# abiswas-odu/Disco

Hardware: AMD Instinct MI355X
Metric: overlaps/sec (BuildGraph stage), 150 bp reads (higher is better)
Workload: dtype u64; 1 GPU; 50000000 x 150 bp synthetic reads, 30x of 50 x 5000000 bp uniform-random contigs, both strands, error-free, min-overlap 40 (k=39), transitive reduction on, seed 42; reads=50000000, read_len=150, min_overlap=40, parallelism=1 GPU, e_pre=903537181, e_out=45314794, n_contained=4685156, cap_bind_sites=0, asymmetric_pairs=0, probes=5550000000, kmer_hits=2220071992

## Files before the change

### disco_amd/csrc/disco_hip.hip

```cpp
#include <hip/hip_runtime.h>
#include <rocprofiler-sdk-roctx/roctx.h>

#include <algorithm>
#include <atomic>
#include <chrono>
#include <cstdarg>
#include <cstdio>
#include <cstdlib>
#include <cstring>
#include <functional>
#include <fcntl.h>
#include <sys/mman.h>
#include <sys/stat.h>
#include <unistd.h>
#include <string>
#include <memory>
#include <thread>
#include <map>
#include <mutex>
#include <queue>
#include <vector>

#include "../../include/disco_hip.h"
#include "../../include/disco_hip_test.h"
// ... 412 lines not shown
            return DISCO_OK;
        }
    }
    tl_pass.dev_allocs++;
    HIPCHK(c, hipMalloc((void **)p, bytes));
    c->hbm_bytes += bytes;
    c->hbm_peak = std::max(c->hbm_peak, c->hbm_bytes);
    return DISCO_OK;
}

template <typename T>
static void dev_free(disco_ctx *c, T **p, size_t count)
{
    if (*p) {
        if (c->arena.owns(*p)) c->arena.release(*p);
        else {
            tl_pass.dev_frees++;
            (void)hipFree(*p);
        }
        c->hbm_bytes -= std::max<size_t>(count, 1) * sizeof(T);
        *p = nullptr;
    }
}

template <typename T>
static void release(disco_ctx *c, DevBuf<T> &b)
{
    dev_free(c, &b.p, b.cap);
    b.cap = 0;
}

template <typename T>
static int ensure(disco_ctx *c, DevBuf<T> &b, u64 need)
{
    if (b.p && need <= b.cap) return DISCO_OK;
    release(c, b);
    CHK(dev_alloc(c, &b.p, need));
    b.cap = std::max<u64>(need, 1);
    return DISCO_OK;
}

template <typename... T>
static int ensure_group(disco_ctx *c, u64 need, u64 size, DevBuf<T> &...b)
{
    if (((need <= b.cap) && ...)) return DISCO_OK;
    (release(c, b), ...);
    int rc = DISCO_OK;
    ((rc = rc == DISCO_OK ? ensure(c, b, size) : rc), ...);
    if (rc != DISCO_OK) (release(c, b), ...);
    return rc;
}

template <typename T>
static int move_keep(disco_ctx *c, DevBuf<T> &b, u64 ncap, u64 used)
{
    DevBuf<T> q;
    CHK(ensure(c, q, ncap));
    if (b.p && used) HIPCHK(c, hipMemcpyAsync(q.p, b.p, used * sizeof(T), hipMemcpyDeviceToDevice, c->stream));
    HIPCHK(c, hipStreamSynchronize(c->stream));
    release(c, b);
    b = q;
    return DISCO_OK;
}

template <typename T>
static int ensure_keep(disco_ctx *c, DevBuf<T> &b, u64 need, u64 used)
{
    if (b.p && need <= b.cap) return DISCO_OK;
    return move_keep(c, b, need + need / 8, used);
}

template <typename T>
static void adopt(disco_ctx *c, DevBuf<T> &b, DevBuf<T> from)
{
    b = from;
    c->hbm_bytes += b.cap * sizeof(T);
}

template <typename T>
static T *disown(disco_ctx *c, DevBuf<T> &b)
{
    T *p = b.p;
    c->hbm_bytes -= b.cap * sizeof(T);
    b = DevBuf<T>();
    return p;
}

static DiscoView view(const disco_ctx *c)
{
    DiscoView v;
    v.reads = c->d_reads;
    v.len = c->d_len;
    v.n = c->n;
    v.S = c->S;
    v.k = c->k;
    v.ks = c->ks;
    v.m = disco_minimizer_len(c->ks);
    if (const char *e = getenv("DISCO_MINIMIZER_LEN")) {
        const int m = atoi(e);
        if (m >= 1 && (m & 1) && m <= v.m && c->ks - m <= 63) v.m = m;
    }
    v.bkt = c->d_bkt;
    v.ent = c->d_ent;
    v.bshift = c->bshift;
    v.q_lo = c->q_lo;
    v.q_hi = c->q_hi;
    v.ctr = c->d_ctr;
    v.wq = c->d_wq;
    v.full = c->two_class ? c->d_full : nullptr;
    v.ovf = c->two_class ? c->d_ovf : nullptr;
    v.long_ids = c->two_class ? c->d_long_ids : nullptr;
    v.n_long = c->two_class ? (u32)c->n_long : 0u;
    v.SL = c->two_class ? c->S_ext : 0;
    v.tailb = c->two_class ? c->tailb : 0;
    return v;
}

static OwnSet own_set(const disco_ctx *c)
{
    OwnSet o;
    o.otab = c->loci ? c->d_otab : nullptr;
    o.me = c->comm ? (u32)c->comm->rank : 0u;
    o.lo = c->q_lo;
    o.hi = c->q_hi;
    o.list = c->loci ? c->d_order_own : nullptr;
    o.n_own = c->loci ? c->n_own : 0;
    o.ids = c->loci ? c->d_own_ids : nullptr;
    return o;
}

static int settle_keys(disco_ctx *c)
{
    if (c->keys_pending) {
        c->keys_pending = false;
        HIPCHK(c, hipStreamWaitEvent(c->stream, c->ev_keys, 0));
    }
    return DISCO_OK;
}

static int env_int(const char *name, int dflt)
{
    const char *e = getenv(name);
    return e ? atoi(e) : dflt;
}

static int wave_grid(const disco_ctx *c, u64 items, int per_cu = 24)
{
    u64 g = (u64)c->n_cu * per_cu;
    if (items < g) g = items;
    return (int)std::max<u64>(g, 1);
}

template <typename K>
static int wq_grid(disco_ctx *c, K kernel, u64 items, const char *env, int cap = 32)
{
    (void)hipMemsetAsync(c->d_wq, 0, sizeof(u64) * WQ_WORDS, c->stream);
    int per_cu = 0;
    if (hipOccupancyMaxActiveBlocksPerMultiprocessor(&per_cu, kernel, 64, 0) != hipSuccess || per_cu <= 0) per_cu = 16;
    if (per_cu > cap) per_cu = cap;
    per_cu = env_int(env, per_cu);
    u64 g = (u64)c->n_cu * per_cu;
    const u64 chunks = (items + WQ_CHUNK - 1) / WQ_CHUNK;
    if (chunks < g) g = chunks;
    return (int)std::max<u64>(g, 1);
}

template <typename K, typename... A>
static void wq_launch(disco_ctx *c, K kernel, u64 items, const char *env, int cap, A... args)
{
    const int g = wq_grid(c, kernel, items, env, cap);
    hipLaunchKernelGGL(kernel, dim3(g), dim3(64), 0, c->stream, args...);
}

static int flat_grid(const disco_ctx *c, u64 items, int block = 256)
{
    u64 g = (items + block - 1) / block;
    u64 cap = (u64)c->n_cu * 16;
    return (int)std::max<u64>(std::min(g, cap), 1);
}

static int read_counters(disco_ctx *c)
{
    HIPCHK(c, hipMemcpyAsync(c->h_ctr, c->d_ctr, sizeof(c->h_ctr), hipMemcpyDeviceToHost, c->stream));
    HIPCHK(c, hipStreamSynchronize(c->stream));
    return DISCO_OK;
}

static int zero_counter(disco_ctx *c, int idx)
{
    HIPCHK(c, hipMemsetAsync(c->d_ctr + idx, 0, sizeof(u64), c->stream));
    return DISCO_OK;
}

template <typename InT, typename OutT>
static int scan_exclusive_on(disco_ctx *c, hipStream_t st, DevBuf<u64> &tile, u64 *total, const InT *in, u64 n, OutT *out, bool write_total, u64 *total_host)
{
    u64 nt = (n + SCAN_TILE - 1) / SCAN_TILE;
    if (nt == 0) nt = 1;
    CHK(ensure(c, tile, nt));
    hipLaunchKernelGGL((scan_tile_sums_kernel<InT>), dim3((unsigned)nt), dim3(SCAN_BLOCK), 0, st, in, n, tile.p);
    hipLaunchKernelGGL(scan_sums_kernel, dim3(1), dim3(1024), 0, st, tile.p, nt, total);
    hipLaunchKernelGGL((scan_apply_kernel<InT, OutT>), dim3((unsigned)nt), dim3(SCAN_BLOCK), 0, st, in, n, tile.p, out);
    if (write_total) hipLaunchKernelGGL((scan_write_total_kernel<OutT>), dim3(1), dim3(1), 0, st, total, out + n);
    HIPCHK(c, hipGetLastError());
    if (total_host) {
        HIPCHK(c, hipMemcpyAsync(total_host, total, sizeof(u64), hipMemcpyDeviceToHost, st));
        HIPCHK(c, hipStreamSynchronize(st));
    }
    return DISCO_OK;
}

template <typename InT, typename OutT>
static int scan_exclusive(disco_ctx *c, const InT *in, u64 n, OutT *out, bool write_total, u64 *total_host)
{
    return scan_exclusive_on<InT, OutT>(c, c->stream, c->d_tile, c->d_total, in, n, out, write_total, total_host);
}

static void drop_edge_records(disco_ctx *c)
{
    c->rec_e_ready = false;
    release(c, c->d_rec_efile);
    release(c, c->d_rec_subs);
    release(c, c->d_rec_efindex);
}
static void drop_contained_records(disco_ctx *c)
{
    c->rec_c_ready = false;
    c->rec_c_n = 0;
    release(c, c->d_rec_cword);
    release(c, c->d_rec_csup);
    release(c, c->d_rec_cfindex);
}

static void free_graph_state(disco_ctx *c)
{
    drop_edge_records(c);
    drop_contained_records(c);
    release(c, c->d_rec_piece[0]);
    release(c, c->d_rec_piece[1]);
    if (c->keys_pending) {
        c->keys_pending = false;
        if (c->ev_keys) (void)hipEventSynchronize(c->ev_keys);
    }
    release(c, c->d_bkt);
    release(c, c->d_ent);
    release(c, c->d_rec);
    release(c, c->d_rec2);
    release(c, c->d_binx);
    release(c, c->d_best);
    release(c, c->d_hits);
    release(c, c->d_row_start);
    release(c, c->d_row_cnt);
    release(c, c->d_big_list);
    release(c, c->d_big_cnt);
    release(c, c->d_slow_list);
    release(c, c->d_runs);
    c->runs_n = 0;
    c->runs_lpr = 0;
    release(c, c->d_contained);
    release(c, c->d_cbits);
    release(c, c->d_dropbits);
    release(c, c->d_drop_node);
    release(c, c->d_drop_key);
    release(c, c->d_adj_ref);
    release(c, c->d_adj_own);
    release(c, c->d_adj_spare);
    release(c, c->d_start_tmp);
    release(c, c->d_ocnt);
    release(c, c->d_okey);
    release(c, c->d_meta_ord);
    release(c, c->d_asked);
    release(c, c->d_oslot);
    release(c, c->d_order_own);
    c->d_order_used = nullptr;
    c->d_adj = nullptr;
    release(c, c->d_extra_cnt);
    release(c, c->d_extra_node);
    release(c, c->d_extra_key);
    release(c, c->d_half);
    release(c, c->d_hcnt);
    release(c, c->d_wide);
    release(c, c->d_n_wide);
    c->adj_total = 0;
    release(c, c->d_out_valid);
    release(c, c->d_ch_comp);
    release(c, c->d_ch_links);
    release(c, c->d_ch_dead);
    release(c, c->d_ch_first);
    release(c, c->d_ch_res_pos);
    release(c, c->d_ch_res_slot);
    c->ch_res_n = 0;
    release(c, c->d_ptext);
    c->ptext_bytes = 0;
    c->ptext_off.clear();
    release(c, c->d_text);
    c->text_bytes = 0;
    release(c, c->d_ctext);
    c->ctext_bytes = 0;
    c->ctext_off.clear();
    c->ch_ready = false;
    release(c, c->d_out_pos);
    release(c, c->d_out_src);
    release(c, c->d_out_ent);
    c->n_out = c->out_used = 0;
    c->flags_pending = false;
    c->adj_imported = false;
    c->T = 0;
    release(c, c->d_x16a);
    release(c, c->d_x16b);
    release(c, c->d_req_flat);
    release(c, c->d_req_s);
    release(c, c->d_req_r);
    release(c, c->d_rdeg_s);
    release(c, c->d_rdeg_r);
    release(c, c->d_rdata_s);
// ... 2527 lines not shown
    if (!c) return DISCO_E_ARG;
    if (c->phase < 5) return fail(c, DISCO_E_STATE, "disco_symmetrize: select edges first");
    HIPCHK(c, hipSetDevice(c->device));
    CHK(twin_check(c, full ? 0 : c->q_lo, full ? c->n : c->q_hi));
    if (n_asym) *n_asym = c->asym_local;
    c->phase = 6;
    return DISCO_OK;
}

int disco_merge_extras(disco_ctx *c)
{
    if (!c) return DISCO_E_ARG;
    if (c->phase < 6) return fail(c, DISCO_E_STATE, "disco_merge_extras: symmetrize first");
    HIPCHK(c, hipSetDevice(c->device));
    return merge_extras(c);
}

int disco_build_edges(disco_ctx *c, uint64_t *n_pre)
{
    if (!c) return DISCO_E_ARG;
    CHK(disco_select_edges(c));
    CHK(disco_symmetrize(c, 1, nullptr));
    CHK(merge_extras(c));
    if (n_pre) *n_pre = c->adj_total / 2;
    return DISCO_OK;
}

int disco_adjacency_size(disco_ctx *c, uint64_t *n_entries)
{
    if (!c || !n_entries) return DISCO_E_ARG;
    if (c->phase < 5) return fail(c, DISCO_E_STATE, "disco_adjacency_size: select edges first");
    *n_entries = c->adj_total;
    return DISCO_OK;
}

int disco_export_adjacency(disco_ctx *c, void *d_deg_u32, void *d_entries_u64)
{
    if (!c || !d_deg_u32) return DISCO_E_ARG;
    if (c->phase < 5 || c->adj_imported) return fail(c, DISCO_E_STATE, "disco_export_adjacency: needs the locally selected edges");
    HIPCHK(c, hipSetDevice(c->device));
    const u64 nq = c->q_hi - c->q_lo;
    ph_begin(c, DISCO_PH_CSR);
    if (nq) hipLaunchKernelGGL(deg_from_ref_kernel, dim3(flat_grid(c, nq)), dim3(256), 0, c->stream, c->d_adj_ref, c->q_lo, c->q_hi, (u32 *)d_deg_u32);
    HIPCHK(c, hipGetLastError());
    if (nq && c->adj_total && d_entries_u64) {
        CHK(ensure(c, c->d_start_tmp, c->n + 1));
        u64 *start = c->d_start_tmp;
        u64 total = 0;
        int rc = scan_exclusive<u32, u64>(c, (const u32 *)d_deg_u32, nq, start, true, &total);
        if (rc == DISCO_OK && total != c->adj_total) rc = fail(c, DISCO_E_STATE, "disco_export_adjacency: degree sum %llu != %llu", (unsigned long long)total, (unsigned long long)c->adj_total);
        if (rc == DISCO_OK) hipLaunchKernelGGL(rows_gather_kernel, dim3(wave_grid(c, nq, 16)), dim3(64), 0, c->stream, c->d_adj, c->d_adj_ref, c->q_lo, c->q_hi, start, (u64 *)d_entries_u64,
                                              (c->phase == 5 && c->prm.max_substitutions != 0) ? 0ull : (u64)ADJ_FLAG);
        hipError_t e = hipStreamSynchronize(c->stream);
        CHK(rc);
        if (e != hipSuccess) return fail(c, DISCO_E_HIP, "disco_export_adjacency: %s", hipGetErrorString(e));
    }
    ph_end(c, DISCO_PH_CSR);
    HIPCHK(c, hipStreamSynchronize(c->stream));
    ph_collect(c);
    return DISCO_OK;
}





int disco_import_adjacency(disco_ctx *c, const void *d_deg_u32_all, const void *d_entries_u64_all, uint64_t n_entries_all)
{
    if (!c || !d_deg_u32_all) return DISCO_E_ARG;
    if (c->phase < 5) return fail(c, DISCO_E_STATE, "disco_import_adjacency: select edges first");
    HIPCHK(c, hipSetDevice(c->device));
    CHK(ensure(c, c->d_start_tmp, c->n + 1));
    u64 *start = c->d_start_tmp;
    u64 total = 0;
    CHK((scan_exclusive<u32, u64>(c, (const u32 *)d_deg_u32_all, c->n, start, true, &total)));
    if (total != n_entries_all)
        return fail(c, DISCO_E_ARG, "disco_import_adjacency: degrees sum to %llu but %llu entries were passed", (unsigned long long)total, (unsigned long long)n_entries_all);
    CHK(ensure(c, c->d_adj_own, total));
    c->d_adj = c->d_adj_own;
    c->adj_total = total;
    if (total) HIPCHK(c, hipMemcpyAsync(c->d_adj, d_entries_u64_all, total * 8, hipMemcpyDeviceToDevice, c->stream));
    if (c->n) hipLaunchKernelGGL(ref_from_start_kernel, dim3(flat_grid(c, c->n)), dim3(256), 0, c->stream, start, (const u32 *)d_deg_u32_all, c->n, c->d_adj_ref);
    HIPCHK(c, hipGetLastError());
    HIPCHK(c, hipStreamSynchronize(c->stream));
    c->adj_imported = true;
    c->tr_big_counted = false;
    c->adj_span = total;
    c->half_complete = false;
    c->phase = 5;
    return DISCO_OK;
}




int disco_transitive_mark(disco_ctx *c)
{
    DISCO_TRACE("disco_transitive_mark");
    if (!c) return DISCO_E_ARG;
    if (c->phase < 6) return fail(c, DISCO_E_STATE, "disco_transitive_mark: build edges first");
    HIPCHK(c, hipSetDevice(c->device));
    const u64 nq = c->q_hi - c->q_lo;
    HIPCHK(c, hipMemsetAsync(c->d_n_big, 0, sizeof(u32), c->stream));
    CHK(zero_counter(c, CTR_OVERFLOW));
    const bool counted_nodes = c->tr_big_counted && c->q_lo == 0 && c->q_hi == c->n && !getenv("DISCO_COUNT_BIG_ROWS");
    const bool tr_small = env_int("DISCO_TR_SMALL", counted_nodes && c->h_ctr[CTR_TR_MID] * 100 <= nq ? 1 : 0) != 0 && counted_nodes;
    if (counted_nodes) {
        const u64 need = c->h_ctr[tr_small ? CTR_TR_MID : CTR_TR_BIG] + 1024;
        if (need > 0xFFFFFFFFull) return fail(c, DISCO_E_CAPACITY, "more than 2^32 big nodes");
        CHK(grow_big_lists(c, need));
    } else
        CHK(ensure_big_cap(c, nullptr, c->d_adj_ref, TR_CAP));
    c->use_half = !getenv("DISCO_NO_HALF");
    const u32 all_flags = (c->adj_imported || !c->use_half || c->q_lo != 0 || c->q_hi != c->n) ? 1u : 0u;
    const bool lists = c->use_half && !all_flags;
    TrArgs a;
    CHK(tr_args_begin(c, &a, lists));
    a.order = (c->d_order_used && c->order_q_lo == c->q_lo && c->order_q_hi == c->q_hi && !c->adj_imported && !getenv("DISCO_TR_NO_ORDER")) ? c->d_order_used : nullptr;
    a.all_flags = all_flags;
    ph_begin(c, DISCO_PH_TRMARK);
    if (nq) wq_launch(c, tr_pick(false, false, tr_small, lists), nq, "DISCO_TR_WAVES", 32, a);
    ph_end(c, DISCO_PH_TRMARK);
    HIPCHK(c, hipGetLastError());
    u32 n_big = 0;
    HIPCHK(c, hipMemcpyAsync(&n_big, c->d_n_big, sizeof(u32), hipMemcpyDeviceToHost, c->stream));
    c->n_wide = 0;
    if (c->use_half) HIPCHK(c, hipMemcpyAsync(&c->n_wide, c->d_n_wide, sizeof(u32), hipMemcpyDeviceToHost, c->stream));
    CHK(read_counters(c));
    ph_collect(c);
    if (c->h_ctr[CTR_OVERFLOW]) return fail(c, DISCO_E_CAPACITY, "transitive marking: big-node list overflow (%u nodes)", n_big);
    if (n_big) {
        CHK(tr_big_nodes(c, &a, n_big, false, "big nodes"));
        if (c->h_ctr[CTR_OVERFLOW]) return fail(c, DISCO_E_CAPACITY, "transitive marking (big nodes): list overflow");
    }
    if (n_big && c->use_half) HIPCHK(c, hipMemcpy(&c->n_wide, c->d_n_wide, sizeof(u32), hipMemcpyDeviceToHost));
    c->flags_pending = false;
    c->phase = 7;
    return DISCO_OK;
}


int disco_emit_edges(disco_ctx *c, uint64_t *n_out)
{
    DISCO_TRACE("disco_emit_edges");
    if (!c) return DISCO_E_ARG;
    if (c->phase < 7) return fail(c, DISCO_E_STATE, "disco_emit_edges: run disco_transitive_mark first");
    HIPCHK(c, hipSetDevice(c->device));
    drop_edge_records(c);
    const u64 nq = c->q_hi - c->q_lo;
    ph_begin(c, DISCO_PH_EMIT);
    const int grid = wq_grid(c, emit_kernel<false>, nq, "DISCO_EMIT_WAVES");
    const u64 n_push = c->dist_active ? c->n_push_r : 0;
    const int grid_push = (int)std::max<u64>(std::min<u64>((n_push + 63) / 64, (u64)c->n_cu * 16), 1);
    const u64 nwaves = (u64)grid * 2 + (n_push ? (u64)grid_push : 0);
    u64 want = std::max<u64>(2 * nq, 1024) + n_push + nwaves * EMIT_CHUNK;
    for (int attempt = 0; attempt < 6; attempt++) {
        CHK(ensure_group(c, want, want, c->d_out_src, c->d_out_ent));
        HIPCHK(c, hipMemsetAsync(c->d_bump, 0, sizeof(u64), c->stream));
        const bool half_emit = c->use_half && c->half_complete;
        const bool dense = half_emit && c->half_selfdel && !c->dist_active;
        if (half_emit && c->half_selfdel && !dense) return fail(c, DISCO_E_STATE, "disco_emit_edges: self-delimiting lists under a communicator");
        c->out_dense = dense;
        if (half_emit && nq) {
            EmitHalfArgs h;
            h.v = view(c);
            h.ref = c->d_adj_ref;
            h.adj = c->d_adj;
            h.half = c->d_half;
            h.hcnt = dense ? nullptr : (const u32 *)c->d_hcnt;
            h.out_src = c->d_out_src;
            h.out_ent = c->d_out_ent;
            h.out_cap = c->d_out_src.cap;
            h.bump = c->d_bump;
            h.local_only = c->dist_active ? 1u : 0u;
            h.own = own_set(c);
            h.order = nullptr;
            if (dense) {
                const int gh = wq_grid(c, emit_half_lists_kernel, (nq + 63) / 64, "DISCO_EMIT_WAVES");
                hipLaunchKernelGGL(emit_half_lists_kernel, dim3(gh), dim3(64), 0, c->stream, h);
            } else {
                const int gh = wq_grid(c, emit_half_kernel, (nq + 63) / 64, "DISCO_EMIT_WAVES");
                hipLaunchKernelGGL(emit_half_kernel, dim3(gh), dim3(64), 0, c->stream, h);
            }
        }
        EmitArgs a;
        a.v = view(c);
        a.ref = c->d_adj_ref;
        a.adj = c->d_adj;
        a.hcnt = half_emit && !dense ? (const u32 *)c->d_hcnt : nullptr;
        a.half = half_emit ? c->d_half : nullptr;
        const bool listed = half_emit && c->n_wide <= c->d_wide.cap;
        a.list = listed ? c->d_wide : nullptr;
        a.n_list = listed ? c->n_wide : 0;
        a.out_src = c->d_out_src;
        a.out_ent = c->d_out_ent;
        a.out_cap = c->d_out_src.cap;
        a.bump = c->d_bump;
        a.local_only = c->dist_active ? 1u : 0u;
        a.own = own_set(c);
        HIPCHK(c, hipMemsetAsync(c->d_wq, 0, sizeof(u64) * WQ_WORDS, c->stream));
        if (nq && !(listed && c->n_wide == 0)) {
            if (dense) hipLaunchKernelGGL(emit_kernel<true>, dim3(grid), dim3(64), 0, c->stream, a);
            else hipLaunchKernelGGL(emit_kernel<false>, dim3(grid), dim3(64), 0, c->stream, a);
        }
        if (n_push) {
            EmitRecvArgs pr;
            pr.items = c->d_push_r;
            pr.n_items = n_push;
            pr.ref = c->d_adj_ref;
            pr.adj = c->d_adj;
            pr.half = c->d_half;
            pr.hcnt = c->d_hcnt;
            pr.out_src = c->d_out_src;
            pr.out_ent = c->d_out_ent;
            pr.out_cap = c->d_out_src.cap;
            pr.bump = c->d_bump;
            pr.wq = c->d_wq;
            HIPCHK(c, hipMemsetAsync(c->d_wq, 0, sizeof(u64) * WQ_WORDS, c->stream));
            hipLaunchKernelGGL(emit_push_recv_kernel, dim3(grid_push), dim3(64), 0, c->stream, pr);
        }
        HIPCHK(c, hipGetLastError());
        u64 used = 0;
        HIPCHK(c, hipMemcpyAsync(&used, c->d_bump, sizeof(u64), hipMemcpyDeviceToHost, c->stream));
        HIPCHK(c, hipStreamSynchronize(c->stream));
        if (used <= c->d_out_src.cap) {
            c->out_used = used;
            break;
        }
        want = used + used / 8 + nwaves * EMIT_CHUNK;
        if (attempt == 5) return fail(c, DISCO_E_CAPACITY, "disco_emit_edges: output buffer could not be sized");
    }
    u64 total = 0;
    if (c->out_dense) {
        total = c->out_used;
        release(c, c->d_out_valid);
        release(c, c->d_out_pos);
    } else if (c->out_used) {
        if (c->out_used > c->d_out_valid.cap || c->out_used + 1 > c->d_out_pos.cap) {
            release(c, c->d_out_valid);
            release(c, c->d_out_pos);
            int rc = ensure(c, c->d_out_valid, c->d_out_src.cap);
            if (rc == DISCO_OK) rc = ensure(c, c->d_out_pos, c->d_out_src.cap + 1);
            if (rc != DISCO_OK) {
                release(c, c->d_out_valid);
                return rc;
            }
        }
        hipLaunchKernelGGL(emit_valid_kernel, dim3(flat_grid(c, c->out_used)), dim3(256), 0, c->stream, c->d_out_src, c->out_used, c->d_out_valid);
        CHK((scan_exclusive<u8, u64>(c, c->d_out_valid, c->out_used, c->d_out_pos, true, nullptr)));
        HIPCHK(c, hipMemcpyAsync(&total, c->d_total, sizeof(u64), hipMemcpyDeviceToHost, c->stream));
    }
    ph_end(c, DISCO_PH_EMIT);
    HIPCHK(c, hipStreamSynchronize(c->stream));
    ph_collect(c);
    c->n_out = total;
    if (n_out) *n_out = total;
    c->phase = 8;
    return DISCO_OK;
}

int disco_transitive_reduce(disco_ctx *c, uint64_t *n_out)
{
    CHK(disco_transitive_mark(c));
    return disco_emit_edges(c, n_out);
}

int disco_run_graph(disco_ctx *c)
{
    DISCO_TRACE("disco_run_graph");
    const bool verbose = getenv("DISCO_VERBOSE") != nullptr;
    auto now = [] { return std::chrono::steady_clock::now(); };
    auto ms = [](std::chrono::steady_clock::time_point a, std::chrono::steady_clock::time_point b) { return std::chrono::duration<double, std::milli>(b - a).count(); };
    auto t0 = now();
    CHK(disco_build_index(c));
    auto t1 = now();
    CHK(disco_probe(c));
    auto t2 = now();
    {
        CHK(ensure(c, c->d_contained, c->n_alloc));
        CHK(ensure(c, c->d_cbits, c->n_alloc / 64 + 1));
        CHK(zero_counter(c, CTR_N_CONTAINED));
        ph_begin(c, DISCO_PH_CONTAIN);
        if (c->n) hipLaunchKernelGGL(contain_flags_kernel, dim3(flat_grid(c, c->n)), dim3(256), 0, c->stream, c->d_best, c->n, c->d_contained, c->d_cbits, c->d_ctr);
        HIPCHK(c, hipGetLastError());
        ph_end(c, DISCO_PH_CONTAIN);
        c->contained_count_pending = true;
        c->phase = 4;
        c->crows_pending = c->cgrp_pending = false;
    }
    auto t3 = now();
    CHK(disco_build_edges(c, nullptr));
    auto t4 = now();
    int rc = disco_transitive_reduce(c, nullptr);
    auto t5 = now();
    if (verbose)
        fprintf(stderr, "[disco] host wall ms: index %.1f probe %.1f contain %.1f edges %.1f reduce %.1f\n", ms(t0, t1), ms(t1, t2), ms(t2, t3), ms(t3, t4), ms(t4, t5));
    return rc;
}

static int ensure_host_len(disco_ctx *c)
{
    std::lock_guard<std::mutex> lk(c->h_len_mu);
    if (c->h_len_ok && c->h_len.size() == c->n) return DISCO_OK;
    c->h_len.resize(c->n);
    if (c->n) HIPCHK(c, hipMemcpy(c->h_len.data(), c->d_len, c->n * 2, hipMemcpyDeviceToHost));
    c->h_len_ok = true;
    return DISCO_OK;
}

int64_t disco_fetch_contained(disco_ctx *c, disco_contained_row *out, uint64_t cap)
{
    DISCO_TRACE("disco_fetch_contained");
    if (!c) return DISCO_E_ARG;
    if (c->phase < 4) return fail(c, DISCO_E_STATE, "disco_fetch_contained: run disco_mark_contained first");
    HIPCHK(c, hipSetDevice(c->device));
    const u64 nc = c->n_contained;
    if (!out) return (int64_t)nc;
    if (cap < nc) return fail(c, DISCO_E_ARG, "disco_fetch_contained: need room for %llu rows", (unsigned long long)nc);
    if (nc == 0) return 0;
    auto decode = [&](auto id_of, const u64 *keys_h, const u32 *lens_h) {
        const u16 *hlen = lens_h ? nullptr : c->h_len.data();
        const u32 kk = (u32)c->k;
        parallel_for(nc, [&, hlen, kk, lens_h](u64 b, u64 e_) {
            for (u64 i = b; i < e_; i++) {
                const u64 key = keys_h[i];
                disco_contained_row &r = out[i];
                r.contained = id_of(i);
                r.super = CKEY_SUPER(key);
                r.j = CKEY_J(key);
                r.type = disco_hit_type(CKEY_SUFFIX(key), CKEY_REV(key));
                r.len2 = lens_h ? (lens_h[i] & 0xFFFFu) : hlen[r.contained];
                r.len1 = lens_h ? (lens_h[i] >> 16) : hlen[r.super];
                u32 orient, off;
                disco_map_type(r.type, r.len1, kk, r.j, &orient, &off);
                r.orient = orient;
                r.start = off;
            }
        });
    };
    CHK(start_contained_rows(c, false));
    if (c->crows_pending && c->crows_n == nc) {
        HIPCHK(c, hipEventSynchronize(c->ev_crows));
        const u64 *hkey = (const u64 *)c->h_crows;
        const u32 *hid = (const u32 *)(hkey + c->crows_hcap);
        decode([hid](u64 i) { return (u64)hid[i]; }, hkey, hid + c->crows_hcap);
        return (int64_t)nc;
    }
    CHK(ensure_host_len(c));
    CHK(settle_keys(c));
    DevBuf<u64> pos, ids, keys;
    std::vector<u64> hid(nc), hkey(nc);
    auto gather = [&]() -> int {
        CHK(ensure(c, pos, c->n + 1));
        CHK(ensure(c, ids, nc));
        CHK(ensure(c, keys, nc));
        CHK((scan_exclusive<u8, u64>(c, c->d_contained, c->n, pos, false, nullptr)));
        hipLaunchKernelGGL(contain_rows_kernel, dim3(flat_grid(c, c->n)), dim3(256), 0, c->stream, c->d_best, c->d_contained, pos, c->n, ids, keys);
        HIPCHK(c, hipMemcpyAsync(hid.data(), ids, nc * 8, hipMemcpyDeviceToHost, c->stream));
        HIPCHK(c, hipMemcpyAsync(hkey.data(), keys, nc * 8, hipMemcpyDeviceToHost, c->stream));
        HIPCHK(c, hipStreamSynchronize(c->stream));
        return DISCO_OK;
    };
    const int grc = gather();
    release(c, pos);
    release(c, ids);
    release(c, keys);
    CHK(grc);
    for (u64 i = 0; i < nc; i++)
        if (CKEY_SUPER(hkey[i]) >= c->n || hid[i] >= c->n)
            return fail(c, DISCO_E_STATE, "disco_fetch_contained: row %llu of %llu: read %llu has the key %llx (no containing read)", (unsigned long long)i, (unsigned long long)nc,
                        (unsigned long long)hid[i], (unsigned long long)hkey[i]);
    decode([&hid](u64 i) { return hid[i]; }, hkey.data(), nullptr);
    return (int64_t)nc;
}

int64_t disco_fetch_contained_grouped(disco_ctx *c, disco_contained_row *out, uint64_t cap)
{
    DISCO_TRACE("disco_fetch_contained_grouped");
    if (!c) return DISCO_E_ARG;
    if (c->phase < 4) return fail(c, DISCO_E_STATE, "disco_fetch_contained_grouped: run disco_mark_contained first");
    HIPCHK(c, hipSetDevice(c->device));
    const u64 nc = c->n_contained;
// ... 3305 lines not shown
```

### disco_amd/csrc/disco_kernels.h

```cpp
#ifndef DISCO_KERNELS_H_
#define DISCO_KERNELS_H_

#include "disco_device.h"
#include "readgen.h"

#define PROBE_ROWCAP 512
#define PROBE_SEGW 128
#define PROBE_SEGP (PROBE_SEGW + 64)
#define PROBE_ACAP 32
#define PROBE_CHUNK 4096
#define ES_MID 1024
#define ES_DUPBITS 11
#define ES_DUPTAB (1 << ES_DUPBITS)
#ifndef ES_CAP
#define ES_CAP 256
#endif
#ifndef TR_CAP
#define TR_CAP 256
#endif
#define TR_CAP_SMALL 128
#define VERIFY_SW 8
#define ORDER_BUCKET(key, shift) (((key) * 0x9E3779B1u) >> (shift))
#define SCAN_ITEMS 16
#define SCAN_BLOCK 256
// ... 3916 lines not shown
#if defined(TR_EXP) && TR_EXP >= 1
    const bool fl = lane < d && lane >= 2u && (ht[sent & 63u] != 0x12345u);
#else
    const u32 hs_end = ht[sent];
    const bool fl = keep & (lane < d) & ((hs_end >> 31) != 0u);
#endif
    const bool fr = keep & (lane < d) & !fl;
    const u64 mk = __ballot(fr);
    if (fl && ((!LISTS && (a.all_flags || !a.half)) || __popcll(mk) > HALF_CAP)) a.adj[nd.vs + lane] = e | ADJ_FLAG;
    const u32 nfree = __popcll(mk);
    const bool selfdel = DEFER ? false : (LISTS || (a.half && !a.hcnt));
    if ((LISTS || a.half) && fr) {
        const u32 r = rank_below(mk);
        if (r < HALF_CAP) a.half[(u64)nd.v * HALF_CAP + r] = selfdel ? surv_encode(e, r, nfree) : e;
    }
    if (selfdel) {
        if (nfree - 1u >= (u32)HALF_CAP && lane == 0 && keep) {
            if (nfree == 0) a.half[(u64)nd.v * HALF_CAP] = SURV_NONE;
            else {
                const u32 idx = atomicAdd(a.n_wide, 1u);
                if (idx < a.wide_cap) a.wide_list[idx] = nd.v;
            }
        }
    } else if ((LISTS || a.hcnt) && lane == 0 && keep) {
        a.hcnt[nd.v] = nfree;
        if (nfree > HALF_CAP) {
            const u32 idx = atomicAdd(a.n_wide, 1u);
            if (idx < a.wide_cap) a.wide_list[idx] = nd.v;
        }
    }
    __syncthreads();
}

#ifndef TR_WAVES_PER_SIMD
#define TR_WAVES_PER_SIMD 6
#endif
template <bool BIG, bool DEFER, int CAP = TR_CAP, bool LISTS = false>
__global__ void __launch_bounds__(64, (CAP == TR_CAP_SMALL && !BIG) ? 8 : TR_WAVES_PER_SIMD) transitive_mark_kernel(TrArgs a)
{
    __shared__ u64 s_hkey[BIG ? 1 : 2 * CAP];
    __shared__ u32 s_ent[BIG ? 1 : CAP];
    __shared__ u8 s_state[BIG ? 1 : 2 * CAP];
    __shared__ u64 s_mid[(BIG || DEFER) ? 1 : 64];
    const u32 lane = threadIdx.x;
    const u64 n_items = BIG ? (u64)min(*a.n_big, a.big_cap) : (a.v.q_hi - a.v.q_lo);
    u64 *hkey = s_hkey;
    u32 *sent = s_ent;
    u8 *hstate = s_state;
    if (BIG) {
        u8 *base = (u8 *)a.scratch + (u64)blockIdx.x * (a.hcap * 8 + a.hcap * 4 + a.hcap);
        hkey = (u64 *)base;
        sent = (u32 *)(base + a.hcap * 8);
        hstate = base + a.hcap * 8 + a.hcap * 4;
    }
    const u32 n_last = (u32)(a.v.n - 1);
    const u32 lane8 = lane << 3;
    u64 cbeg = 0, cend = 0;
    u64 rv_chunk = 0;
    u32 v_chunk = 0;
    u32 ccnt = 0;
    auto stage_row = [&](u32 t) {
        TrNodeRegs r;
        const bool ok = t < ccnt;
        const u32 tc = ok ? t : ccnt - 1u;
        const u64 rv = readlane_u64(rv_chunk, tc);
        r.v = (u32)__builtin_amdgcn_readlane((int)v_chunk, (int)tc);
        r.vs = REF_POS(rv);
        r.dfull = ok ? REF_DEG(rv) : 0u;
        r.d = (r.dfull <= 64) ? r.dfull : 0u;
        r.e = *(const u64 *)((const u8 *)(a.adj + r.vs) + (lane < r.d ? lane8 : 0u));
        r.s2 = 0;
        r.r0 = r.r2 = r.p0 = r.p2 = 0;
        return r;
    };
    auto stage_refs = [&](TrNodeRegs &r) {
        r.e &= ~ADJ_FLAG;
        const u32 side0 = ADJ_ORI(readlane_u64(r.e, 0)) >> 1;
        const u64 om = __ballot((ADJ_ORI(r.e) >> 1) != side0);
        r.s2 = om ? (u32)__ffsll((long long)om) - 1u : 0u;
        const u64 e0 = readlane_u64(r.e, 0), e2 = readlane_u64(r.e, r.s2);
        r.r0 = a.ref[min((u32)ADJ_DST(e0), n_last)];
        r.r2 = a.ref[min((u32)ADJ_DST(e2), n_last)];
    };
    auto stage_rows = [&](TrNodeRegs &r) {
        r.r0 = uniform_u64(r.r0);
        r.r2 = uniform_u64(r.r2);
        const u32 d0 = REF_DEG(r.r0), d2 = REF_DEG(r.r2);
        r.p0 = *(const u64 *)((const u8 *)(a.adj + REF_POS(r.r0)) + (lane < d0 ? lane8 : 0u));
        r.p2 = *(const u64 *)((const u8 *)(a.adj + REF_POS(r.r2)) + (lane < d2 ? lane8 : 0u));
    };
#if defined(WQ_SPLIT_ALL)
    WqSplit wqs;
    while (BIG ? wq_grab<1>(a.v.wq, n_items, cbeg, cend) : wq_grab_split(a.v.wq, n_items, cbeg, cend, wqs)) {
#else
    while (BIG ? wq_grab<1>(a.v.wq, n_items, cbeg, cend) : wq_grab(a.v.wq, n_items, cbeg, cend)) {
#endif
    if (BIG) {
        for (u64 it = cbeg; it < cend; it++) {
            const u64 v = a.big_list[it];
            const u32 d = REF_DEG(a.ref[v]);
            if (d == 0) continue;
            tr_node<DEFER>(a, v, d, hkey, hstate, sent, (u32)a.hcap - 1, lane);
        }
        continue;
    }
    {
        const u64 idx = cbeg + lane, ic = idx < cend ? idx : cend - 1;
        v_chunk = (u32)(a.order ? ORDER_ID(a.order[ic]) : a.v.q_lo + ic);
        rv_chunk = a.ref[v_chunk];
    }
    ccnt = (u32)(cend - cbeg);
    TrNodeRegs n0 = stage_row(0), n1 = stage_row(1), n2 = stage_row(2), n3;
    stage_refs(n0);
    stage_refs(n1);
    stage_rows(n0);
    u32 n_mid = 0;
    auto step = [&](TrNodeRegs &A, TrNodeRegs &B, TrNodeRegs &C, TrNodeRegs &D, u32 t) {
        stage_rows(B);
        stage_refs(C);
        D = stage_row(t + 3);
        if (A.d != 0)
            tr_node_small<DEFER, LISTS>(a, A, s_hkey, s_state, lane);
        else if (A.dfull != 0) {
            if (!DEFER && A.dfull <= (u32)CAP) {
                if (lane == 0) s_mid[n_mid] = A.v;
                n_mid++;
            } else if (lane == 0) {
                u32 idx = atomicAdd(a.n_big, 1u);
                if (idx < a.big_cap) a.big_list[idx] = A.v;
                else atomicAdd(&a.v.ctr[CTR_OVERFLOW], 1ull);
            }
        }
    };
    for (u32 t = 0; t < ccnt; t += 4) {
        step(n0, n1, n2, n3, t);
        step(n1, n2, n3, n0, t + 1);
        step(n2, n3, n0, n1, t + 2);
        step(n3, n0, n1, n2, t + 3);
    }
    if (!DEFER && n_mid) {
        __syncthreads();
        for (u32 x = 0; x < n_mid; x++) {
            const u64 v = s_mid[x];
            const u32 dv = REF_DEG(a.ref[v]);
            u32 hc = 64;
            while (hc < 2 * dv) hc <<= 1;
            tr_node<DEFER>(a, v, dv, hkey, hstate, sent, hc - 1, lane);
        }
        __syncthreads();
    }
    }
}

#define EMIT_CHUNK 256
struct EmitArgs {
    DiscoView v;
    const u64 *ref;
    const u64 *adj;
    const u32 *hcnt;
    const u64 *half;
    const u64 *list;
    u64 n_list;
    u64 *out_src;
    u64 *out_ent;
    u64 out_cap;
    u64 *bump;
    u32 local_only;
    OwnSet own;
};

struct EmitStage {
    u64 *src, *ent;
    u32 staged;
    __device__ __forceinline__ void flush(u64 *bump, u64 *out_src, u64 *out_ent, u64 out_cap, u32 lane)
    {
        if (!staged) return;
        __syncthreads();
        u64 base = 0;
        if (lane == 0) base = atomicAdd(bump, (u64)staged);
        base = uniform_u64(base);
        for (u32 i = lane; i < staged; i += 64)
            if (base + i < out_cap) {
                out_src[base + i] = src[i];
                out_ent[base + i] = ent[i];
            }
        __syncthreads();
        staged = 0;
    }
    __device__ __forceinline__ void append(u64 mk, bool keep, u64 v, u64 e, u64 *bump, u64 *out_src, u64 *out_ent, u64 out_cap, u32 lane)
    {
        const u32 kc = __popcll(mk);
        if (!kc) return;
        if (staged + kc > EMIT_CHUNK) flush(bump, out_src, out_ent, out_cap, lane);
        if (keep) {
            const u32 i = staged + rank_below(mk);
            src[i] = v;
            ent[i] = e;
        }
        staged += kc;
    }
};

template <bool DENSE>
__global__ void __launch_bounds__(64) emit_kernel(EmitArgs a)
{
    __shared__ u64 s_src[DENSE ? EMIT_CHUNK : 1], s_ent[DENSE ? EMIT_CHUNK : 1];
    EmitStage st{s_src, s_ent, 0u};
    const u32 lane = threadIdx.x;
    const bool selfdel = a.half && !a.hcnt;
    u64 chunk_base = 0;
    u32 chunk_used = EMIT_CHUNK;
    bool have_chunk = false;
    auto close_chunk = [&]() {
        if (have_chunk)
            for (u32 i = chunk_used + lane; i < EMIT_CHUNK; i += 64)
                if (chunk_base + i < a.out_cap) a.out_src[chunk_base + i] = ~0ull;
    };
    u64 cbeg = 0, cend = 0;
    while (wq_grab(a.v.wq, a.list ? a.n_list : a.own.count(), cbeg, cend))
    for (u64 it = cbeg; it < cend; it++) {
        const u64 v = a.list ? a.list[it] : a.own.node(it);
        if (!a.own.mine(v)) continue;
        if (a.hcnt && a.hcnt[v] <= HALF_CAP) continue;
        const u64 rv = a.ref[v];
        const u32 d = REF_DEG(rv);
        if (d == 0) continue;
        if (selfdel) {
            const u64 *hv = a.half + v * HALF_CAP;
            if (surv_len(hv[0], hv[1], hv[2], hv[3]) <= HALF_CAP) continue;
        }
        const u64 vs = REF_POS(rv);
        const u32 Lv = a.v.len[v];
        for (u32 s0 = 0; s0 < d; s0 += 64) {
            const u32 s = s0 + lane;
            bool keep = false;
            u64 e = 0;
            if (s < d) {
                e = a.adj[vs + s];
                const u64 w = ADJ_DST(e);
                if (v < w && !(e & ADJ_FLAG) && (!a.local_only || a.own.mine(w))) {
                    const u32 Lw = ADJ_DLEN(e);
                    const u64 twin = ADJ_MAKE(Lw + ADJ_OFF(e) - Lv, v, disco_twin_orient(ADJ_ORI(e)), Lv);
                    const u64 *hw = a.half + w * HALF_CAP;
                    const u32 cw = a.hcnt ? a.hcnt[w] : selfdel ? surv_len(hw[0], hw[1], hw[2], hw[3]) : HALF_CAP + 1;
                    if (cw <= HALF_CAP) {
                        for (u32 r = 0; r < cw; r++) keep |= (surv_entry(hw[r]) == twin);
                    } else {
                        const u64 rw = a.ref[w];
                        const u64 *roww = a.adj + REF_POS(rw);
                        const int ti = adj_find(roww, REF_DEG(rw), twin);
                        keep = (ti >= 0) && !(roww[ti] & ADJ_FLAG);
                    }
                }
            }
            const u64 mk = __ballot(keep);
            if (DENSE) {
                st.append(mk, keep, v, e & ~ADJ_FLAG, a.bump, a.out_src, a.out_ent, a.out_cap, lane);
                continue;
            }
            const u32 cnt = __popcll(mk);
            if (cnt) {
                if (chunk_used + cnt > EMIT_CHUNK) {
                    close_chunk();
                    u64 base = 0;
                    if (lane == 0) base = atomicAdd(a.bump, (u64)EMIT_CHUNK);
                    chunk_base = uniform_u64(base);
                    chunk_used = 0;
                    have_chunk = true;
                }
                if (keep) {
                    const u64 pos = chunk_base + chunk_used + rank_below(mk);
                    if (pos < a.out_cap) {
                        a.out_src[pos] = v;
                        a.out_ent[pos] = e & ~ADJ_FLAG;
                    }
                }
                chunk_used += cnt;
            }
        }
    }
    if (DENSE) st.flush(a.bump, a.out_src, a.out_ent, a.out_cap, lane);
    else close_chunk();
}

struct EmitHalfArgs {
    DiscoView v;
    const u64 *ref;
    const u64 *adj;
    const u64 *half;
    const u32 *hcnt;
    u64 *out_src;
    u64 *out_ent;
    u64 out_cap;
    u64 *bump;
    u32 local_only;
    OwnSet own;
    const u64 *order;
};

__global__ void __launch_bounds__(64) emit_half_kernel(EmitHalfArgs a)
{
    const u32 lane = threadIdx.x;
    u64 chunk_base = 0;
    u32 chunk_used = EMIT_CHUNK;
    bool have_chunk = false;
    auto close_chunk = [&]() {
        if (have_chunk)
            for (u32 i = chunk_used + lane; i < EMIT_CHUNK; i += 64)
                if (chunk_base + i < a.out_cap) a.out_src[chunk_base + i] = ~0ull;
    };
    const u64 nq = a.own.count();
    u64 cbeg = 0, cend = 0;
    while (wq_grab(a.v.wq, (nq + 63) / 64, cbeg, cend))
    for (u64 blk = cbeg; blk < cend; blk++) {
        const bool live = blk * 64 + lane < nq;
        const u64 v = a.order ? ORDER_ID(a.order[live ? blk * 64 + lane : 0]) : a.own.node_by_id(live ? blk * 64 + lane : 0);
        const u32 cnt = live ? a.hcnt[v] : 0u;
        const u32 Lv = live ? (u32)a.v.len[v] : 0u;
#pragma unroll
        for (u32 r = 0; r < HALF_CAP; r++) {
            bool keep = false;
            u64 e = 0;
            if (cnt <= HALF_CAP && r < cnt) {
                e = a.half[v * HALF_CAP + r];
                const u64 w = ADJ_DST(e);
                if (v < w && (!a.local_only || a.own.otab || w < a.own.hi)) {
                    const u64 twin = ADJ_MAKE(ADJ_DLEN(e) + ADJ_OFF(e) - Lv, v, disco_twin_orient(ADJ_ORI(e)), Lv);
                    const u32 cw = a.hcnt[w];
                    if (cw <= HALF_CAP) {
                        const ulonglong2 *hw = (const ulonglong2 *)(a.half + w * HALF_CAP);
                        const ulonglong2 h0 = hw[0], h1 = hw[1];
                        keep = (cw > 0 && h0.x == twin) || (cw > 1 && h0.y == twin) || (cw > 2 && h1.x == twin) || (cw > 3 && h1.y == twin);
                    } else {
                        const u64 rw = a.ref[w];
                        const u64 *roww = a.adj + REF_POS(rw);
                        const int ti = adj_find(roww, REF_DEG(rw), twin);
                        keep = (ti >= 0) && !(roww[ti] & ADJ_FLAG);
                    }
                }
            }
            const u64 mk = __ballot(keep);
            const u32 kc = __popcll(mk);
            if (kc) {
                if (chunk_used + kc > EMIT_CHUNK) {
                    close_chunk();
                    u64 base = 0;
                    if (lane == 0) base = atomicAdd(a.bump, (u64)EMIT_CHUNK);
                    chunk_base = uniform_u64(base);
                    chunk_used = 0;
                    have_chunk = true;
                }
                if (keep) {
                    const u64 pos = chunk_base + chunk_used + rank_below(mk);
                    if (pos < a.out_cap) {
                        a.out_src[pos] = v;
                        a.out_ent[pos] = e;
                    }
                }
                chunk_used += kc;
            }
        }
    }
    close_chunk();
}

__global__ void __launch_bounds__(64) emit_half_lists_kernel(EmitHalfArgs a)
{
    __shared__ u64 s_src[EMIT_CHUNK], s_ent[EMIT_CHUNK];
    EmitStage st{s_src, s_ent, 0u};
    const u32 lane = threadIdx.x;
    const u64 nq = a.own.count();
    u64 cbeg = 0, cend = 0;
    while (wq_grab(a.v.wq, (nq + 63) / 64, cbeg, cend))
    for (u64 blk = cbeg; blk < cend; blk++) {
        const bool live = blk * 64 + lane < nq;
        const u64 v = a.order ? ORDER_ID(a.order[live ? blk * 64 + lane : 0]) : a.own.node_by_id(live ? blk * 64 + lane : 0);
        const ulonglong2 *hv = (const ulonglong2 *)(a.half + v * HALF_CAP);
        const ulonglong2 o0 = hv[0], o1 = hv[1];
        const u64 rv = a.ref[v];
        const u32 Lv = (u32)a.v.len[v];
        const u64 own[HALF_CAP] = {o0.x, o0.y, o1.x, o1.y};
        u32 cnt = (live && REF_DEG(rv) != 0) ? surv_len(own[0], own[1], own[2], own[3]) : 0u;
        if (cnt > HALF_CAP) cnt = 0;
#pragma unroll
        for (u32 r = 0; r < HALF_CAP; r++) {
            bool keep = false;
            const u64 e = surv_entry(own[r]);
            const u64 w = ADJ_DST(e);
            if (r < cnt && v < w && (!a.local_only || a.own.otab || w < a.own.hi)) {
                const u64 twin = ADJ_MAKE(ADJ_DLEN(e) + ADJ_OFF(e) - Lv, v, disco_twin_orient(ADJ_ORI(e)), Lv);
                const ulonglong2 *hw = (const ulonglong2 *)(a.half + w * HALF_CAP);
                const ulonglong2 h0 = hw[0], h1 = hw[1];
                if (surv_len(h0.x, h0.y, h1.x, h1.y) <= HALF_CAP) keep = surv_has(h0.x, h0.y, h1.x, h1.y, twin);
                else {
                    const u64 rw = a.ref[w];
                    const u64 *roww = a.adj + REF_POS(rw);
                    const int ti = adj_find(roww, REF_DEG(rw), twin);
                    keep = (ti >= 0) && !(roww[ti] & ADJ_FLAG);
                }
            }
            st.append(__ballot(keep), keep, v, e, a.bump, a.out_src, a.out_ent, a.out_cap, lane);
        }
    }
    st.flush(a.bump, a.out_src, a.out_ent, a.out_cap, lane);
}

__global__ void emit_valid_kernel(const u64 *__restrict__ out_src, u64 n, u8 *__restrict__ valid)
{
    u64 i = (u64)blockIdx.x * blockDim.x + threadIdx.x;
    for (; i < n; i += (u64)gridDim.x * blockDim.x) valid[i] = out_src[i] != ~0ull;
}

__global__ void emit_compact32_kernel(const u64 *__restrict__ out_src, const u64 *__restrict__ out_ent, const u8 *__restrict__ valid,
                                      const u64 *__restrict__ pos, u64 n, u32 *__restrict__ dst_src, u64 *__restrict__ dst_ent)
{
    u64 i = (u64)blockIdx.x * blockDim.x + threadIdx.x;
    for (; i < n; i += (u64)gridDim.x * blockDim.x)
        if (valid[i]) {
            dst_src[pos[i]] = (u32)out_src[i];
            dst_ent[pos[i]] = out_ent[i];
        }
}

__global__ void emit_src32_kernel(const u64 *__restrict__ out_src, u64 n, u32 *__restrict__ dst_src)
{
    u64 i = (u64)blockIdx.x * blockDim.x + threadIdx.x;
    for (; i < n; i += (u64)gridDim.x * blockDim.x) dst_src[i] = (u32)out_src[i];
}

__global__ void emit_compact_kernel(const u64 *__restrict__ out_src, const u64 *__restrict__ out_ent, const u8 *__restrict__ valid,
                                    const u64 *__restrict__ pos, u64 n, u64 *__restrict__ dst_src, u64 *__restrict__ dst_ent)
{
    u64 i = (u64)blockIdx.x * blockDim.x + threadIdx.x;
    for (; i < n; i += (u64)gridDim.x * blockDim.x)
        if (valid[i]) {
            dst_src[pos[i]] = out_src[i];
            dst_ent[pos[i]] = out_ent[i];
        }
}

__global__ void edge_subs_kernel(const u64 *__restrict__ out_src, const u64 *__restrict__ out_ent, const u8 *__restrict__ valid,
                                 const u64 *__restrict__ pos, u64 n, const u64 *__restrict__ reads, const u16 *__restrict__ len, int S,
                                 u16 *__restrict__ subs)
{
    u64 i = (u64)blockIdx.x * blockDim.x + threadIdx.x;
    for (; i < n; i += (u64)gridDim.x * blockDim.x)
        if (!valid || valid[i]) {
            const u64 src = out_src[i], e = out_ent[i];
            const int l1 = (int)len[src], l2 = (int)ADJ_DLEN(e), off = (int)ADJ_OFF(e), ovl = l1 - off;
            const u32 o = ADJ_ORI(e);
            const u32 rev = (o == 1 || o == 2);
            subs[pos ? pos[i] : i] = (u16)seg_mismatches<false>(reads + src * S, reads + ADJ_DST(e) * S, S, l2, o >= 2 ? off : 0, o >= 2 ? 0 : l2 - ovl, ovl, rev);
        }
}

__device__ __forceinline__ u32 uf_load(const u32 *p) { return __hip_atomic_load(p, __ATOMIC_RELAXED, __HIP_MEMORY_SCOPE_AGENT); }

__device__ __forceinline__ u32 uf_find(u32 *parent, u32 x)
{
    for (;;) {
        const u32 p = uf_load(&parent[x]);
        if (p == x) return x;
        const u32 g = uf_load(&parent[p]);
        if (g != p) __hip_atomic_store(&parent[x], g, __ATOMIC_RELAXED, __HIP_MEMORY_SCOPE_AGENT);
        x = p;
    }
}

__global__ void uf_init_kernel(u32 *parent, u64 n)
{
    u64 i = (u64)blockIdx.x * blockDim.x + threadIdx.x;
    for (; i < n; i += (u64)gridDim.x * blockDim.x) parent[i] = (u32)i;
}

__global__ void uf_hook_kernel(const u64 *__restrict__ out_src, const u64 *__restrict__ out_ent, const u8 *__restrict__ valid, u64 n_slots, u32 *parent)
{
    u64 i = (u64)blockIdx.x * blockDim.x + threadIdx.x;
    for (; i < n_slots; i += (u64)gridDim.x * blockDim.x) {
        if (valid && !valid[i]) continue;
        u32 a = (u32)out_src[i], b = (u32)ADJ_DST(out_ent[i]);
        for (;;) {
            a = uf_find(parent, a);
            b = uf_find(parent, b);
            if (a == b) break;
            if (a < b) {
                const u32 t = a;
                a = b;
                b = t;
            }
            if (atomicCAS(&parent[a], a, b) == a) break;
        }
    }
}

__global__ void uf_compress_kernel(u32 *parent, u64 n)
{
    u64 i = (u64)blockIdx.x * blockDim.x + threadIdx.x;
    for (; i < n; i += (u64)gridDim.x * blockDim.x) {
        u32 r = (u32)i;
        while (parent[r] != r) r = parent[r];
        parent[i] = r;
    }
}

#define UF_SLOTS 1024u
__global__ void __launch_bounds__(256) uf_count_kernel(const u64 *__restrict__ out_src, const u8 *__restrict__ valid, u64 n_slots, const u32 *__restrict__ parent, u32 *cnt)
{
    __shared__ u32 s_key[UF_SLOTS], s_val[UF_SLOTS];
    for (u32 x = threadIdx.x; x < UF_SLOTS; x += blockDim.x) {
        s_key[x] = 0xFFFFFFFFu;
        s_val[x] = 0u;
    }
    __syncthreads();
    u64 i = (u64)blockIdx.x * blockDim.x + threadIdx.x;
    for (; i < n_slots; i += (u64)gridDim.x * blockDim.x)
        if (!valid || valid[i]) {
            const u32 root = parent[(u32)out_src[i]];
            u32 idx = (root * 0x9E3779B1u) >> 22;
            bool placed = false;
            for (int t = 0; t < 8 && !placed; t++) {
                const u32 old = atomicCAS(&s_key[idx], 0xFFFFFFFFu, root);
                if (old == 0xFFFFFFFFu || old == root) {
                    atomicAdd(&s_val[idx], 1u);
                    placed = true;
                } else
                    idx = (idx + 1u) & (UF_SLOTS - 1u);
            }
            if (!placed) atomicAdd(&cnt[root], 1u);
        }
    __syncthreads();
    for (u32 x = threadIdx.x; x < UF_SLOTS; x += blockDim.x)
        if (s_val[x]) atomicAdd(&cnt[s_key[x]], s_val[x]);
}

__global__ void uf_big_kernel(const u32 *__restrict__ cnt, u64 n, u32 thr, u64 *list, u32 *n_list, u32 cap)
{
    u64 i = (u64)blockIdx.x * blockDim.x + threadIdx.x;
    for (; i < n; i += (u64)gridDim.x * blockDim.x)
        if (cnt[i] >= thr) {
            const u32 k = atomicAdd(n_list, 1u);
            if (k < cap) list[k] = (i << 32) | cnt[i];
        }
}

__global__ void uf_assign_kernel(const u64 *__restrict__ pairs, u32 n_pairs, u16 *cfile)
{
    u32 i = blockIdx.x * blockDim.x + threadIdx.x;
    if (i < n_pairs) cfile[pairs[i] >> 32] = (u16)(pairs[i] & 0xFFFF);
}

__global__ void uf_edge_file_kernel(const u64 *__restrict__ out_src, const u8 *__restrict__ valid, const u64 *__restrict__ pos, u64 n_slots,
                                    const u32 *__restrict__ parent, const u16 *__restrict__ cfile, u32 n_files, u16 *edge_file)
{
    u64 i = (u64)blockIdx.x * blockDim.x + threadIdx.x;
    for (; i < n_slots; i += (u64)gridDim.x * blockDim.x)
        if (!valid || valid[i]) {
            const u32 r = parent[(u32)out_src[i]];
// ... 92 lines not shown
```

Before: 11.37 billion overlaps/s.

## Stage dense half-list emission per 4-wave workgroup with shared bump flush

The dense emit_half_lists_kernel now runs 4-wave workgroups. Each wave stages survivors into its own slice of a larger LDS buffer, and the workgroup flushes with a single atomicAdd on the global bump counter when any slice nears capacity. Work is grabbed in multi-block units per atomic on the work queue. The goal is fewer global atomics and larger, more coalesced output writes. In exchange it adds workgroup barriers every unit, uses more LDS per block (which may lower occupancy), and reserves more output slack per workgroup.

Measured after the change: 11.52 billion overlaps/s, median of 5. 1.3% higher.

```diff
diff --git a/disco_amd/csrc/disco_hip.hip b/disco_amd/csrc/disco_hip.hip
--- a/disco_amd/csrc/disco_hip.hip
+++ b/disco_amd/csrc/disco_hip.hip
@@ -588,15 +588,15 @@
 }
 
 template <typename K>
-static int wq_grid(disco_ctx *c, K kernel, u64 items, const char *env, int cap = 32)
+static int wq_grid(disco_ctx *c, K kernel, u64 items, const char *env, int cap = 32, int block = 64, u64 chunk = WQ_CHUNK)
 {
     (void)hipMemsetAsync(c->d_wq, 0, sizeof(u64) * WQ_WORDS, c->stream);
     int per_cu = 0;
-    if (hipOccupancyMaxActiveBlocksPerMultiprocessor(&per_cu, kernel, 64, 0) != hipSuccess || per_cu <= 0) per_cu = 16;
+    if (hipOccupancyMaxActiveBlocksPerMultiprocessor(&per_cu, kernel, block, 0) != hipSuccess || per_cu <= 0) per_cu = 16 * 64 / block;
     if (per_cu > cap) per_cu = cap;
     per_cu = env_int(env, per_cu);
     u64 g = (u64)c->n_cu * per_cu;
-    const u64 chunks = (items + WQ_CHUNK - 1) / WQ_CHUNK;
+    const u64 chunks = (items + chunk - 1) / chunk;
     if (chunks < g) g = chunks;
     return (int)std::max<u64>(g, 1);
 }
@@ -3430,15 +3430,18 @@
     const int grid = wq_grid(c, emit_kernel<false>, nq, "DISCO_EMIT_WAVES");
     const u64 n_push = c->dist_active ? c->n_push_r : 0;
     const int grid_push = (int)std::max<u64>(std::min<u64>((n_push + 63) / 64, (u64)c->n_cu * 16), 1);
-    const u64 nwaves = (u64)grid * 2 + (n_push ? (u64)grid_push : 0);
-    u64 want = std::max<u64>(2 * nq, 1024) + n_push + nwaves * EMIT_CHUNK;
+    const bool half_emit = c->use_half && c->half_complete;
+    const bool dense = half_emit && c->half_selfdel && !c->dist_active;
+    if (half_emit && c->half_selfdel && !dense) return fail(c, DISCO_E_STATE, "disco_emit_edges: self-delimiting lists under a communicator");
+    c->out_dense = dense;
+    const int gh = dense ? wq_grid(c, emit_half_lists_kernel, (nq + 63) / 64, "DISCO_EMIT_WAVES", 32, 64 * EMIT_WG_WAVES, EMIT_WG_WAVES * EMIT_WG_GRAB)
+                         : wq_grid(c, emit_half_kernel, (nq + 63) / 64, "DISCO_EMIT_WAVES");
+    const u64 slack = ((u64)grid + (n_push ? (u64)grid_push : 0)) * EMIT_CHUNK + (u64)gh * (dense ? EMIT_WG_STAGE : EMIT_CHUNK);
+    u64 want = std::max<u64>(2 * nq, 1024) + n_push + slack;
     for (int attempt = 0; attempt < 6; attempt++) {
         CHK(ensure_group(c, want, want, c->d_out_src, c->d_out_ent));
         HIPCHK(c, hipMemsetAsync(c->d_bump, 0, sizeof(u64), c->stream));
-        const bool half_emit = c->use_half && c->half_complete;
-        const bool dense = half_emit && c->half_selfdel && !c->dist_active;
-        if (half_emit && c->half_selfdel && !dense) return fail(c, DISCO_E_STATE, "disco_emit_edges: self-delimiting lists under a communicator");
-        c->out_dense = dense;
+        HIPCHK(c, hipMemsetAsync(c->d_wq, 0, sizeof(u64) * WQ_WORDS, c->stream));
         if (half_emit && nq) {
             EmitHalfArgs h;
             h.v = view(c);
@@ -3453,13 +3456,8 @@
             h.local_only = c->dist_active ? 1u : 0u;
             h.own = own_set(c);
             h.order = nullptr;
-            if (dense) {
-                const int gh = wq_grid(c, emit_half_lists_kernel, (nq + 63) / 64, "DISCO_EMIT_WAVES");
-                hipLaunchKernelGGL(emit_half_lists_kernel, dim3(gh), dim3(64), 0, c->stream, h);
-            } else {
-                const int gh = wq_grid(c, emit_half_kernel, (nq + 63) / 64, "DISCO_EMIT_WAVES");
-                hipLaunchKernelGGL(emit_half_kernel, dim3(gh), dim3(64), 0, c->stream, h);
-            }
+            if (dense) hipLaunchKernelGGL(emit_half_lists_kernel, dim3(gh), dim3(64 * EMIT_WG_WAVES), 0, c->stream, h);
+            else hipLaunchKernelGGL(emit_half_kernel, dim3(gh), dim3(64), 0, c->stream, h);
         }
         EmitArgs a;
         a.v = view(c);
@@ -3505,7 +3503,7 @@
             c->out_used = used;
             break;
         }
-        want = used + used / 8 + nwaves * EMIT_CHUNK;
+        want = used + used / 8 + slack;
         if (attempt == 5) return fail(c, DISCO_E_CAPACITY, "disco_emit_edges: output buffer could not be sized");
     }
     u64 total = 0;
diff --git a/disco_amd/csrc/disco_kernels.h b/disco_amd/csrc/disco_kernels.h
--- a/disco_amd/csrc/disco_kernels.h
+++ b/disco_amd/csrc/disco_kernels.h
@@ -4092,7 +4092,9 @@
     }
 }
 
+#ifndef EMIT_CHUNK
 #define EMIT_CHUNK 256
+#endif
 struct EmitArgs {
     DiscoView v;
     const u64 *ref;
@@ -4304,15 +4306,56 @@
     close_chunk();
 }
 
-__global__ void __launch_bounds__(64) emit_half_lists_kernel(EmitHalfArgs a)
-{
-    __shared__ u64 s_src[EMIT_CHUNK], s_ent[EMIT_CHUNK];
-    EmitStage st{s_src, s_ent, 0u};
-    const u32 lane = threadIdx.x;
+#ifndef EMIT_WG_STAGE
+#define EMIT_WG_STAGE 2048
+#endif
+#define EMIT_WG_WAVES 4u
+#define EMIT_WG_PART (EMIT_WG_STAGE / EMIT_WG_WAVES)
+#define EMIT_WG_TRIP (64u * HALF_CAP)
+#define EMIT_WG_GRAB 16u
+static_assert(EMIT_WG_PART >= EMIT_WG_TRIP, "an empty part must hold a whole trip");
+__global__ void __launch_bounds__(64 * EMIT_WG_WAVES) emit_half_lists_kernel(EmitHalfArgs a)
+{
+    __shared__ u64 s_src[EMIT_WG_STAGE], s_ent[EMIT_WG_STAGE];
+    __shared__ u64 s_word;
+    __shared__ u32 s_cnt[2][EMIT_WG_WAVES];
+    const u32 lane = threadIdx.x & 63u, wave = threadIdx.x >> 6;
     const u64 nq = a.own.count();
-    u64 cbeg = 0, cend = 0;
-    while (wq_grab(a.v.wq, (nq + 63) / 64, cbeg, cend))
-    for (u64 blk = cbeg; blk < cend; blk++) {
+    const u64 nblk = (nq + 63) / 64, nunits = (nblk + EMIT_WG_WAVES - 1) / EMIT_WG_WAVES;
+    u64 *const p_src = s_src + wave * EMIT_WG_PART, *const p_ent = s_ent + wave * EMIT_WG_PART;
+    u32 mine = 0;
+    u32 par = 0;
+    if (threadIdx.x < 2 * EMIT_WG_WAVES) (&s_cnt[0][0])[threadIdx.x] = 0;
+    auto flush = [&]() {
+        u32 before = 0, total = 0;
+        for (u32 w = 0; w < EMIT_WG_WAVES; w++) {
+            const u32 c = uniform_u32(s_cnt[par][w]);
+            if (w < wave) before += c;
+            total += c;
+        }
+        if (threadIdx.x == 0) s_word = atomicAdd(a.bump, (u64)total);
+        __syncthreads();
+        const u64 base = uniform_u64(s_word) + before;
+        for (u32 i = lane; i < mine; i += 64)
+            if (base + i < a.out_cap) {
+                a.out_src[base + i] = p_src[i];
+                a.out_ent[base + i] = p_ent[i];
+            }
+        mine = 0;
+        __syncthreads();
+    };
+    for (;;) {
+        if (threadIdx.x == 0) s_word = atomicAdd(a.v.wq, (u64)EMIT_WG_GRAB);
+        __syncthreads();
+        const u64 ubeg = uniform_u64(s_word);
+        if (ubeg >= nunits) break;
+        const u64 uend = ubeg + EMIT_WG_GRAB < nunits ? ubeg + EMIT_WG_GRAB : nunits;
+    for (u64 unit = ubeg; unit < uend; unit++, par ^= 1u) {
+        __syncthreads();
+        u32 fullest = 0;
+        for (u32 w = 0; w < EMIT_WG_WAVES; w++) fullest = max(fullest, uniform_u32(s_cnt[par][w]));
+        if (fullest + EMIT_WG_TRIP > EMIT_WG_PART) flush();
+        const u64 blk = unit * EMIT_WG_WAVES + wave;
         const bool live = blk * 64 + lane < nq;
         const u64 v = a.order ? ORDER_ID(a.order[live ? blk * 64 + lane : 0]) : a.own.node_by_id(live ? blk * 64 + lane : 0);
         const ulonglong2 *hv = (const ulonglong2 *)(a.half + v * HALF_CAP);
@@ -4339,10 +4382,18 @@
                     keep = (ti >= 0) && !(roww[ti] & ADJ_FLAG);
                 }
             }
-            st.append(__ballot(keep), keep, v, e, a.bump, a.out_src, a.out_ent, a.out_cap, lane);
-        }
-    }
-    st.flush(a.bump, a.out_src, a.out_ent, a.out_cap, lane);
+            const u64 mk = __ballot(keep);
+            if (keep) {
+                const u32 i = mine + rank_below(mk);
+                p_src[i] = v;
+                p_ent[i] = e;
+            }
+            mine += __popcll(mk);
+        }
+        if (lane == 0) s_cnt[par ^ 1u][wave] = mine;
+    }
+    }
+    flush();
 }
 
 __global__ void emit_valid_kernel(const u64 *__restrict__ out_src, u64 n, u8 *__restrict__ valid)
```
